# valette/FROG

Measured on AMD Instinct MI355X. Metric: registration iterations/sec (linear+deformable), higher is better.
Workload: dtype f32

## Files before the change

### frog_amd/csrc/device/ctx.h

```cpp
#pragma once

#include <hip/hip_runtime.h>

#include <cstdint>
#include <cstdio>
#include <cstring>
#include <string>
#include <memory>
#include <vector>

#include "../../../include/frog_hip.h"
#include "dev_buf.h"

namespace frog {

extern thread_local std::string g_last_error;

inline int fail(int code, const std::string &msg)
{
    g_last_error = msg;
    return code;
}

#define FROG_HIP_CHECK(expr)                                                            \
// ... 71 lines not shown
    std::shared_ptr<DevBuf<float4>> kept_u;
    std::shared_ptr<DevBuf<float4>> kept;
    bool retired = false;
};

}

struct frog_ctx {
    int device = 0;
    hipStream_t stream = nullptr;
    bool own_stream = false;
    frog_options opt{};

    uint32_t nI = 0, ib = 0, ie = 0;
    uint64_t P = 0;
    uint32_t own_pt_begin = 0, own_pt_end = 0;
    uint64_t L_own = 0;
    uint64_t L_recs = 0;
    std::vector<uint32_t> poff;
    std::vector<uint64_t> img_link_begin;

    frog::DevBuf<float4> pos;
    frog::DevBuf<frog::P3> pos2;
    frog::DevBuf<frog::P3> pos2_spec;
    frog::DevBuf<uint32_t> d_poff;
    frog::DevBuf<uint64_t> ref_rowptr;
    frog::DevBuf<uint32_t> ref_link;
    std::vector<uint32_t> h_old_of_new, h_new_of_old;
    frog::DevBuf<uint32_t> new_of_old;
    frog::DevBuf<frog::Tile> tiles;
    frog::DevBuf<frog::LinkRec> recs;
    frog::DevBuf<uint32_t> recs32;
    frog::RecFormat rec_format{};
    uint32_t n_tiles = 0;
    frog::DevBuf<uint32_t> img_tile_ptr;
    std::vector<uint32_t> h_img_tile_ptr;
    uint32_t n_sub = 1, n_groups = frog::N_XCD;
    uint32_t group_begin[frog::MAX_GROUPS + 1] = {};
    frog::DevBuf<double> tile_partial;
    frog::DevBuf<long long> tile_counts;
    frog::DevBuf<float4> group_sums;
    frog::DevBuf<float4> point_sums;
    frog::DevBuf<uint32_t> tile_order;
    frog::DevBuf<frog::Tile> tiles_bo;
    uint32_t n_order_blocks = 0;
    bool fused_sweep = false;
    bool fused_forced = false;

    frog::DevBuf<float4> em;
    frog::DevBuf<frog::EmDerived> emd;
    frog::DevBuf<frog::EmFast> emf;
    frog::DevBuf<float> samples;
    frog::DevBuf<unsigned char> em_guess;
    static constexpr int SEL_RING_MAX = 96;
    static constexpr int SEL_LOW_WATER = 3;
    int sel_ring = 2;
    frog::DevBuf<uint32_t> sample_ord[SEL_RING_MAX];
    frog::DevBuf<uint32_t> sample_count[SEL_RING_MAX];
    frog::DevBuf<uint2> sample_ends[SEL_RING_MAX];
    uint64_t sel_consumed = 0;
    uint64_t sel_produced = 0;
    int sel_used = 0;
    hipStream_t side = nullptr;
    hipStream_t setup_stream = nullptr;
    hipEvent_t setup_fork = nullptr, setup_join = nullptr;
    bool setup_pending = false;
    bool setup_deferred = false;
    hipEvent_t energy_copied = nullptr;
    bool xyz2_exported = false;
    hipEvent_t sel_done[SEL_RING_MAX] = {};
    hipEvent_t ord_read[SEL_RING_MAX] = {};
    frog::DevBuf<uint32_t> mt_state;
    std::vector<uint32_t> h_virtual;
    frog::DevBuf<uint32_t> d_virtual;
    int sample_cap = 0;

    frog::DevBuf<double> mat;
    frog::DevBuf<double> energy;
    frog::DevBuf<double> energy_blocks;
    frog::DevBuf<double> img_energy;
    frog::DevBuf<unsigned int> energy_ticket;
    double *h_energy = nullptr;
    double *h_energy_dev = nullptr;
    uint64_t scalar_seq = 0;

    bool deformable = false;
    frog::GridGeom geom{};
    frog::DevBuf<float4> coeff;
    frog::DevBuf<float4> grad;
    frog::DevBuf<float4> gradf;
    frog::DevBuf<float4> grad_spare;
    frog::DevBuf<uint32_t> lat_mask;
    frog::DevBuf<uint32_t> lat_inactive;
    frog::DevBuf<float4> ucoeff, ugrad, ugrad_spare;
    frog::DevBuf<double> gridsum;
    frog::DevBuf<uint32_t> perm;
    frog::DevBuf<uint32_t> key_ptr;
    frog::DevBuf<uint32_t> key_cursor;
    frog::DevBuf<uint32_t> key_counts, brick_ptr_scratch, scan_sums;
    frog::DevBuf<unsigned char> scatter_blocks;
    frog::DevBuf<unsigned char> scatter_blocks_tmp;
    frog::DevBuf<uint32_t> len_hist;
    uint32_t n_scatter_blocks = 0;
    frog::DevBuf<float> bounds_scratch;
    frog::DevBuf<unsigned int> stray;
    uint32_t stray_parity = 0;
// ... 110 lines not shown
```

### frog_amd/csrc/device/frog_hip.hip

```cpp

#include "ctx.h"
#include <hip/hip_ext.h>
#include "prep.h"
#include "k_links.hip.h"
#include "k_stats.hip.h"
#include "k_grid.hip.h"
#include "k_cull.hip.h"
#include "k_ransac.hip.h"
#include "k_reforder.hip.h"
#include "k_refchain.hip.h"
#include "similarity.h"

#include <atomic>
#include <chrono>
#include <cmath>
#include <cstdlib>
#include <random>
#include <limits>
#include <new>

namespace frog {
thread_local std::string g_last_error;
constexpr int BOUNDS_BLOCKS = 256;
void set_last_error(const std::string &s) { g_last_error = s; }
// ... 828 lines not shown
        const int n_slices = [&] {
            const char *e = getenv("FROG_TILE_SLICES");
            const int v = e ? atoi(e) : (c->ie - c->ib >= 64u ? 2 : 8);
            return v < 1 ? 1 : v > 64 ? 64 : v;
        }();
        for (int sl = 0; sl < n_slices; sl++)
            for (uint32_t i = c->ib; i < c->ie; i++) {
                const uint32_t tb = lay.img_tile_ptr[i], nt = lay.img_tile_ptr[i + 1] - tb;
                for (uint32_t j = 0; j < nt; j++)
                    if ((int)(((size_t)j * N_XCD * n_slices / nt) % n_slices) == sl) lists[(size_t)j * N_XCD / nt].push_back(tb + j);
            }
        size_t rounds = 0;
        for (auto &l : lists) rounds = std::max(rounds, l.size());
        std::vector<uint32_t> order(std::max<size_t>(1, rounds * N_XCD), 0xFFFFFFFFu);
        for (int x = 0; x < N_XCD; x++)
            for (size_t r = 0; r < lists[x].size(); r++) order[r * N_XCD + x] = lists[x][r];
        c->n_order_blocks = (uint32_t)(rounds * N_XCD);
        CREATE_CHECK(c->tile_order.upload(order, s));
        {
            std::vector<Tile> bo(order.size(), Tile{});
            for (size_t b = 0; b < order.size(); b++) if (order[b] != 0xFFFFFFFFu) bo[b] = lay.tiles[order[b]];
            CREATE_CHECK(c->tiles_bo.upload(bo, s));
            CREATE_CHECK(hipStreamSynchronize(s));
        }
        CREATE_CHECK(hipStreamSynchronize(s));
        uint32_t widest = 0;
        for (uint32_t g = 0; g < c->n_groups; g++) widest = std::max(widest, c->group_begin[g + 1] - c->group_begin[g]);
        const char *fe = getenv("FROG_SWEEP_FUSED");
        c->fused_sweep = c->n_sub == 1 && c->n_tiles > 0 && widest <= (uint32_t)EMD_LDS_IMAGES && sweep_lds_images(c) <= 64u
                         && !(fe && fe[0] == '0');
        c->fused_forced = fe && fe[0] == '1';
    }
    CREATE_CHECK(c->tile_partial.alloc((size_t)std::max(1u, c->n_tiles) * c->n_groups * LINEAR_SUMS));
    CREATE_CHECK(c->tile_counts.alloc((size_t)std::max(1u, c->n_tiles) * c->n_groups * 2));
    CREATE_CHECK(c->group_sums.alloc((size_t)N_XCD * std::max(1u, c->own_pt_end - c->own_pt_begin)));
    CREATE_CHECK(c->img_counts.alloc((size_t)c->n_owned() * 2));

    std::vector<float4> hem(c->nI, make_float4(10.f, 300.f, 0.5f, 0.f));
    CREATE_CHECK(c->em.upload(hem, s));
    CREATE_CHECK(c->emd.alloc(c->nI));
    CREATE_CHECK(c->emf.alloc(c->nI));
    c->h_virtual.resize(c->n_owned());
    uint32_t cap = 1;
    for (uint32_t i = c->ib; i < c->ie; i++) {
        uint64_t v = lay.img_link_begin[i + 1] - lay.img_link_begin[i];
        c->h_virtual[i - c->ib] = (uint32_t)v;
        cap = std::max<uint32_t>(cap, (uint32_t)std::min<uint64_t>(v, (uint64_t)o->stats_max_size));
    }
    c->sample_cap = (int)cap;
    CREATE_CHECK(c->d_virtual.upload(c->h_virtual, s));
    CREATE_CHECK(c->samples.alloc((size_t)c->n_owned() * cap));
    CREATE_CHECK(c->em_guess.alloc((size_t)c->n_owned() * 4 * EM_GUESS_BATCHES));
    CREATE_CHECK(hipMemsetAsync(c->em_guess.p, 0, c->em_guess.bytes(), s));
    c->sel_ring = 80;
    static_assert(80 <= frog_ctx::SEL_RING_MAX, "the ring's buffers are fixed arrays of frog_ctx");
    while (c->sel_ring > 2 && (size_t)c->sel_ring * c->n_owned() * cap * 12 > ((size_t)1 << 30)) c->sel_ring--;
    for (int b = 0; b < c->sel_ring; b++) {
        CREATE_CHECK(c->sample_ord[b].alloc((size_t)c->n_owned() * cap));
        CREATE_CHECK(c->sample_ends[b].alloc((size_t)c->n_owned() * cap));
        CREATE_CHECK(c->sample_count[b].alloc(c->n_owned()));
        CREATE_CHECK(hipMemsetAsync(c->sample_count[b].p, 0, c->sample_count[b].bytes(), s));
        CREATE_CHECK(hipEventCreateWithFlags(&c->ord_read[b], hipEventDisableTiming));
        CREATE_CHECK(hipEventCreateWithFlags(&c->sel_done[b], hipEventDisableTiming));
    }
    {
        int lo = 0, hi = 0;
        CREATE_CHECK(hipDeviceGetStreamPriorityRange(&lo, &hi));
        const bool high = c->sel_ring < 3;
        CREATE_CHECK(hipStreamCreateWithPriority(&c->side, hipStreamNonBlocking, high ? hi : lo));
    }
    CREATE_CHECK(hipEventCreateWithFlags(&c->energy_copied, hipEventDisableTiming));
    CREATE_CHECK(hipStreamCreateWithFlags(&c->setup_stream, hipStreamNonBlocking));
    CREATE_CHECK(hipEventCreateWithFlags(&c->setup_fork, hipEventDisableTiming));
    CREATE_CHECK(hipEventCreateWithFlags(&c->setup_join, hipEventDisableTiming));
    {
        std::vector<uint32_t> st((size_t)c->n_owned() * MT_WORDS);
        uint32_t x[MT_WORDS];
        x[0] = 0u;
        for (int k = 1; k < MT_N; k++) x[k] = 1812433253u * (x[k - 1] ^ (x[k - 1] >> 30)) + (uint32_t)k;
        x[MT_N] = MT_N;
        for (uint32_t i = 0; i < c->n_owned(); i++) std::memcpy(&st[(size_t)i * MT_WORDS], x, sizeof x);
        CREATE_CHECK(c->mt_state.upload(st, s));
    }

    std::vector<double> hm((size_t)c->nI * 16, 0.0);
    for (uint32_t i = 0; i < c->nI; i++) for (int k = 0; k < 4; k++) hm[(size_t)i * 16 + 5 * k] = 1.0;
    CREATE_CHECK(c->mat.upload(hm, s));
    CREATE_CHECK(c->energy.alloc(4));
    CREATE_CHECK(c->energy_blocks.alloc(2 * ENERGY_BLOCKS));
    CREATE_CHECK(c->img_energy.alloc(2 * (size_t)std::max(1u, c->n_owned())));
    CREATE_CHECK(c->energy_ticket.alloc(2));
    CREATE_CHECK(hipMemsetAsync(c->energy_ticket.p, 0, 2 * sizeof(unsigned int), s));
    CREATE_CHECK(hipMemsetAsync(c->energy.p, 0, c->energy.bytes(), s));
    CREATE_CHECK(c->stray.alloc(3));
    CREATE_CHECK(hipMemsetAsync(c->stray.p, 0, 3 * sizeof(unsigned int), s));
    CREATE_CHECK(c->bounds_scratch.alloc((size_t)BOUNDS_BLOCKS * 6 + 6));
    em_derive_kernel<<<div_up(c->nI, 256), 256, 0, s>>>(c->em.p, c->emd.p, c->emf.p, c->nI, c->fast_theta());
    CREATE_CHECK(hipGetLastError());
    if (const char *e = getenv("FROG_CULL")) c->cull_enabled = atoi(e) != 0;
    if (!(c->cull_enabled && c->opt.inlier_threshold >= 1e-3f) && !c->fused_forced) c->fused_sweep = false;
    if (const char *e = getenv("FROG_WEIGHT_EXACT")) c->exact_weights = atoi(e) != 0;
    if (const char *e = getenv("FROG_WEIGHT_GENERAL")) c->general_weights = atoi(e) != 0;
    c->ref_order = o->reference_order != 0;
    if (const char *e = getenv("FROG_REFERENCE_ORDER")) c->ref_order = atoi(e) != 0;
    if (const char *e = getenv("FROG_K11_F64")) c->k11_f64 = atoi(e) != 0;
    if (c->ref_order) { c->cull_enabled = false; c->exact_weights = true; c->fused_sweep = false; }
// ... 263 lines not shown
                                                                             ctx->perm.p, n, ctx->ib, to_dev(ctx->geom), apply,
                                                                             with_disp ? ctx->pos2_snap.p : nullptr, ctx->disp_part.p,
                                                                             after_step ? ctx->grad.p : nullptr, ctx->energy.p,
                                                                             ctx->opt.guarantee_diffeomorphism,
                                                                             ctx->disp_allow.p, ctx->cull_state.p, host_scalars, scalar_seq, trailer,
                                                                             pt_xcd ? nb : 0u);
            if (with_disp) ctx->disp_n = ctx->disp_own_n = div_up(n, 256);
        }
        trailer = nullptr;
        ctx->disp_others = false;
        if (out == ctx->pos2.p) ctx->disp_current = with_disp;
        else { ctx->disp_spec = with_disp; ctx->disp_current = false; }
    }
    if (trailer) slab_trailer_kernel<<<1, 1, 0, ctx->stream>>>(ctx->energy.p, trailer);
    FROG_HIP_CHECK(hipGetLastError());
    if (apply) { ctx->pos_b_stale = true; ctx->rc_valid = false; }
    return FROG_OK;
}

int frog_transform_points_local(frog_ctx *ctx, int apply)
{
    CTX_GUARD(ctx);
    const uint32_t n = ctx->own_pt_end - ctx->own_pt_begin;
    if (!n) return FROG_OK;
    if (ctx->xyz2_fresh && !apply) {
        ctx->xyz2_fresh = false; ctx->res_valid = false;
        ctx->disp_current = ctx->disp_spec;
        if (ctx->n_owned() == ctx->nI && !ctx->xyz2_exported && ctx->pos2_spec.n == ctx->pos2.n) {
            std::swap(ctx->pos2.p, ctx->pos2_spec.p);
            std::swap(ctx->pos2.cap, ctx->pos2_spec.cap);
            return FROG_OK;
        }
        FROG_HIP_CHECK(hipMemcpyAsync(ctx->pos2.p + ctx->own_pt_begin, ctx->pos2_spec.p + ctx->own_pt_begin,
                                      (size_t)n * sizeof(P3), hipMemcpyDeviceToDevice, ctx->stream));
        return FROG_OK;
    }
    ctx->xyz2_fresh = false; ctx->res_valid = false;
    return launch_transform(ctx, ctx->pos2.p, apply);
}

int frog_transform_points(frog_ctx *ctx, int apply) { return frog_transform_points_local(ctx, apply); }

int frog_update_stats_local(frog_ctx *ctx)
{
    CTX_GUARD(ctx);
    const uint32_t nO = ctx->n_owned();
    const uint32_t cap = (uint32_t)ctx->sample_cap;
    hipStream_t s = ctx->stream;
    const int cur = (int)(ctx->sel_consumed % (uint64_t)ctx->sel_ring);
    FROG_HIP_CHECK(hipStreamWaitEvent(s, ctx->sel_done[cur], 0));
    {
        Span span(ctx, FROG_K_STATS);
        sample_distance_kernel<<<dim3(div_up(cap, 256), nO), 256, 0, s>>>(
            ctx->sample_ends[cur].p, ctx->sample_count[cur].p, cap, ctx->pos2.p, ctx->samples.p);
        FROG_HIP_CHECK(hipGetLastError());
        em_scan_kernel<<<nO, EM_THREADS, 0, s>>>(ctx->samples.p, ctx->sample_count[cur].p, cap, ctx->ib, ctx->em.p,
                                                 ctx->opt.stats_max_iterations, ctx->opt.stats_epsilon, ctx->em_guess.p);
        FROG_HIP_CHECK(hipGetLastError());
    }
    FROG_HIP_CHECK(hipEventRecord(ctx->ord_read[cur], s));
    ctx->sel_used = cur;
    ctx->sel_consumed++;
    if (ctx->sel_produced - ctx->sel_consumed < (uint64_t)std::min((int)frog_ctx::SEL_LOW_WATER, ctx->sel_ring - 1))
        while (ctx->sel_produced - ctx->sel_consumed < (uint64_t)(ctx->sel_ring - 1)) {
            const int rc = produce_selection(ctx);
            if (rc) return rc;
            if (ctx->sel_ring > 8) break;
        }
    if (ctx->ib > 0) FROG_HIP_CHECK(hipMemsetAsync(ctx->em.p, 0, (size_t)ctx->ib * sizeof(float4), s));
    if (ctx->ie < ctx->nI)
        FROG_HIP_CHECK(hipMemsetAsync(ctx->em.p + ctx->ie, 0, (size_t)(ctx->nI - ctx->ie) * sizeof(float4), s));
    return FROG_OK;
}

int frog_stats_publish(frog_ctx *ctx)
{
    CTX_GUARD(ctx);
    stats_publish_kernel<<<dim3(div_up(ctx->nI, 64), 2), 64, 0, ctx->stream>>>(ctx->em.p, ctx->emd.p, ctx->emf.p, ctx->nI, ctx->opt.inlier_threshold, ctx->fast_theta(), ctx->cut_now.p,
                                                                       ctx->deformable ? 0 : 1);
    if (!ctx->deformable) ctx->cull_need_build = true;
    ctx->cull_check_due = true;
    FROG_HIP_CHECK(hipGetLastError());
    return FROG_OK;
}

int frog_update_stats(frog_ctx *ctx)
{
    if (ctx && !ctx->whole_group())
        return fail(FROG_E_STATE, "context owns a sub-range of images: use frog_update_stats_local + all-reduce + frog_stats_publish");
    int rc = frog_update_stats_local(ctx);
    if (rc) return rc;
    if (ctx->helper) {
        frog_ctx *h = ctx->helper;
        const size_t n = ctx->own_pt_end - ctx->own_pt_begin;
        FROG_HIP_CHECK(hipMemcpyAsync(h->pos2.p + ctx->own_pt_begin, ctx->pos2.p + ctx->own_pt_begin, n * sizeof(P3),
                                      hipMemcpyDeviceToDevice, ctx->stream));
        rc = frog_update_stats_local(h);
        if (rc) return rc;
        FROG_HIP_CHECK(hipMemcpyAsync(ctx->em.p, h->em.p, (size_t)ctx->nf * sizeof(float4), hipMemcpyDeviceToDevice, ctx->stream));
    }
    return frog_stats_publish(ctx);
}

int frog_ransac(frog_ctx *ctx, const frog_model *m, uint32_t image, const frog_ransac_options *o, int64_t *n_inliers)
{
    CTX_GUARD(ctx);
    if (!m || !o) return fail(FROG_E_INVALID, "null argument");
    if (image < ctx->ib || image >= ctx->ie) return fail(FROG_E_INVALID, "image not owned by this context");
    if (m->n_images != ctx->nI || m->point_offset[ctx->nI] != ctx->P) return fail(FROG_E_INVALID, "model does not match the context");
    if (ctx->deformable) return fail(FROG_E_STATE, "RANSAC after deformable set-up");
// ... 1048 lines not shown
    if (hipGetDeviceCount(&ndev) != hipSuccess || ndev < 1) return fail(FROG_E_NODEVICE, "no HIP device");
    if (device < 0 || device >= ndev) return fail(FROG_E_INVALID, "device index out of range");
    FROG_HIP_CHECK(hipSetDevice(device));
    if (!n) return FROG_OK;
    DevBuf<double> df, dw;
    FROG_HIP_CHECK(df.alloc(n)); FROG_HIP_CHECK(dw.alloc(4 * n));
    FROG_HIP_CHECK(hipMemcpy(df.p, f, n * sizeof(double), hipMemcpyHostToDevice));
    test_weights_kernel<<<div_up(n, 256), 256>>>(df.p, n, dw.p);
    FROG_HIP_CHECK(hipGetLastError());
    FROG_HIP_CHECK(hipMemcpy(out4n, dw.p, 4 * n * sizeof(double), hipMemcpyDeviceToHost));
    return FROG_OK;
}

int frog_test_cull_ranges(frog_ctx *ctx, uint64_t *ranges, uint64_t *with_election)
{
    CTX_GUARD(ctx);
    if (!ranges || !with_election) return fail(FROG_E_INVALID, "null output");
    *ranges = 0; *with_election = 0;
    if (ctx->cull_builds && ctx->act_cnt.n) {
        std::vector<uint32_t> h(ctx->act_cnt.n);
        FROG_HIP_CHECK(hipMemcpyAsync(h.data(), ctx->act_cnt.p, ctx->act_cnt.bytes(), hipMemcpyDeviceToHost, ctx->stream));
        FROG_HIP_CHECK(hipStreamSynchronize(ctx->stream));
        for (uint32_t v : h) {
            if (v & ~CULL_DUP_BIT) (*ranges)++;
            if (v & CULL_DUP_BIT) (*with_election)++;
        }
    }
    return FROG_OK;
}

int frog_test_stray_points(frog_ctx *ctx, uint64_t *n)
{
    CTX_GUARD(ctx);
    { const int rc_ = join_setup(ctx); if (rc_) return rc_; }
    if (!n) return fail(FROG_E_INVALID, "null output");
    unsigned int v = 0;
    FROG_HIP_CHECK(hipMemcpyAsync(&v, ctx->stray.p + 2, sizeof v, hipMemcpyDeviceToHost, ctx->stream));
    FROG_HIP_CHECK(hipStreamSynchronize(ctx->stream));
    *n = v;
    return FROG_OK;
}

int frog_test_em_refit(frog_ctx *ctx, int term_by_term)
{
    CTX_GUARD(ctx);
    const uint32_t nO = ctx->n_owned(), cap = (uint32_t)ctx->sample_cap;
    const int cur = ctx->sel_used;
    hipStream_t s = ctx->stream;
    if (term_by_term)
        em_kernel<<<nO, 256, 0, s>>>(ctx->samples.p, ctx->sample_count[cur].p, cap, ctx->ib, ctx->em.p,
                                     ctx->opt.stats_max_iterations, ctx->opt.stats_epsilon);
    else
        em_scan_kernel<<<nO, EM_THREADS, 0, s>>>(ctx->samples.p, ctx->sample_count[cur].p, cap, ctx->ib, ctx->em.p,
                                                 ctx->opt.stats_max_iterations, ctx->opt.stats_epsilon, nullptr);
    FROG_HIP_CHECK(hipGetLastError());
    return frog_stats_publish(ctx);
}

int frog_profile_enable(frog_ctx *ctx, int on)
{
    CTX_GUARD(ctx);
    ctx->profiling = (on == 2 || on == 3) ? 2 : (on != 0);
    ctx->profile_stride = on == 3 ? 4 : 1;
    return FROG_OK;
}

int frog_profile_read(frog_ctx *ctx, frog_kernel_time *out, int reset)
{
    CTX_GUARD(ctx);
    FROG_HIP_CHECK(hipStreamSynchronize(ctx->stream));
    for (auto &sp : ctx->spans) {
        float ms = 0.f;
        if (hipEventElapsedTime(&ms, sp.a, sp.b) == hipSuccess) {
            ctx->timed_ms[sp.slot] += (double)ms;
            ctx->timed_n[sp.slot] += 1;
        }
        ctx->free_events.emplace_back(sp.a, sp.b);
    }
    ctx->spans.clear();
    for (int k = 0; k < FROG_K_COUNT_; k++) {
        const uint64_t launches = ctx->timed_n[k] ? std::max(ctx->span_seen[k], ctx->timed_n[k]) : 0;
        ctx->ktime[k].launches = launches;
        ctx->ktime[k].ms_total = ctx->timed_n[k] ? ctx->timed_ms[k] / (double)ctx->timed_n[k] * (double)launches : 0.0;
    }
    if (out) std::memcpy(out, ctx->ktime, sizeof ctx->ktime);
    if (reset) {
        std::memset(ctx->ktime, 0, sizeof ctx->ktime);
        std::memset(ctx->span_seen, 0, sizeof ctx->span_seen);
        std::memset(ctx->timed_ms, 0, sizeof ctx->timed_ms);
        std::memset(ctx->timed_n, 0, sizeof ctx->timed_n);
    }
    return FROG_OK;
}

constexpr int UNPACK_MAX_RANKS = 64;
struct UnpackArgs {
    uint64_t row_begin[UNPACK_MAX_RANKS + 1];
    uint64_t slot_bytes;
    uint32_t world, self;
    uint64_t trailer_off;
    uint32_t sum_mask;
    double *energy, *host_scalars;
    double seq;
};
__global__ __launch_bounds__(256) void unpack_slab_kernel(const P3 *slab, P3 *pos2, const UnpackArgs a, const P3 *snap, uint32_t *disp_part)
{
    __shared__ uint32_t sh[4];
// ... 217 lines not shown
```

### frog_amd/csrc/device/k_stats.hip.h

```cpp
#pragma once

#include "ctx.h"

namespace frog {

constexpr int MT_N = 624;
constexpr int MT_M = 397;
constexpr int MT_WORDS = MT_N + 1;

__device__ __forceinline__ uint32_t mt_twist(uint32_t cur, uint32_t nxt, uint32_t far)
{
    uint32_t y = (cur & 0x80000000u) | (nxt & 0x7fffffffu);
    return far ^ (y >> 1) ^ ((y & 1u) ? 0x9908b0dfu : 0u);
}

constexpr int SELECT_THREADS = 256;

__device__ __forceinline__ void mt_regenerate(uint32_t *x, int tid)
{
    constexpr int LAG = MT_N - MT_M;
    uint32_t a = 0, b = 0, c = 0;
    if (tid < LAG) {
        a = mt_twist(x[tid], x[tid + 1], x[tid + MT_M]);
        b = mt_twist(x[tid + LAG], x[tid + LAG + 1], a);
// ... 87 lines not shown
            uint32_t rank = before + ((below_pk >> (8 * r)) & 0xFFu);
            #pragma unroll
            for (int w = 0; w < SELECT_THREADS / 64; w++) {
                const uint32_t c = row_cnt[r][w];
                if (w < wave) rank += c;
                before += c;
            }
            const uint32_t q = (uint32_t)tid + (uint32_t)(SELECT_THREADS * r);
            if (((keep_bits >> r) & 1u) && rank < need) ord[count + rank] = ordinal + q;
            if (((keep_bits >> r) & 1u) && fills && rank == need - 1) jstar_s = (int)q;
        }
        const bool advance = !fills && idx + n == (uint32_t)MT_N && ordinal + n < vs;
        if (advance && tid < LAG) {
            x[tid] = na;
            x[tid + LAG] = nb;
            if (tid + 2 * LAG < MT_N) x[tid + 2 * LAG] = nc;
        }
        __syncthreads();
        if (fills) {
            const uint32_t jstar = (uint32_t)jstar_s;
            idx += jstar + 1;
            ordinal += jstar + 1;
            count = cap;
            done = true;
        } else {
            count += kept;
            ordinal += n;
            idx = advance ? 0u : idx + n;
        }
    }
    for (int k = tid; k < MT_N; k += SELECT_THREADS) st[k] = x[k];
    if (tid == 0) { st[MT_N] = idx; sample_count[img] = count; }
}

__global__ __launch_bounds__(256) void sample_resolve_kernel(
    const uint32_t *sample_ord, const uint32_t *sample_count, uint32_t cap,
    const uint32_t *poff, uint32_t image_begin, uint32_t own_pt_begin,
    const uint64_t *ref_rowptr, const uint32_t *ref_link, const uint32_t *new_of_old, uint2 *sample_ends)
{
    const uint32_t img = blockIdx.y;
    const uint32_t slot = blockIdx.x * blockDim.x + threadIdx.x;
    if (slot >= sample_count[img]) return;
    const uint32_t image = image_begin + img;
    const uint32_t pb = poff[image] - own_pt_begin, pe = poff[image + 1] - own_pt_begin;
    const uint64_t l = ref_rowptr[pb] + sample_ord[(size_t)img * cap + slot];
    uint32_t lo = pb, hi = pe;
    while (hi - lo > 1) {
        uint32_t mid = (lo + hi) >> 1;
        if (ref_rowptr[mid] <= l) lo = mid; else hi = mid;
    }
    sample_ends[(size_t)img * cap + slot] = make_uint2(new_of_old[lo], ref_link[l]);
}

__global__ __launch_bounds__(256) void sample_distance_kernel(const uint2 *sample_ends, const uint32_t *sample_count, uint32_t cap,
                                                              const P3 *pos2, float *samples)
{
    const uint32_t img = blockIdx.y;
    const uint32_t slot = blockIdx.x * blockDim.x + threadIdx.x;
    if (slot >= sample_count[img]) return;
    const uint2 ends = sample_ends[(size_t)img * cap + slot];
    const P3 a = pos2[ends.x];
    const P3 b = pos2[ends.y];
    const float dx = a.x - b.x, dy = a.y - b.y, dz = a.z - b.z;
    samples[(size_t)img * cap + slot] = sqrtf(dx * dx + dy * dy + dz * dz);
}

__device__ __forceinline__ float chi_pdf_ref(float x)
{
    const float c = 0.797884560802865f;
    const float x2 = x * x;
    const float cx2 = c * x2;
    return (float)((double)cx2 * exp(-0.5 * (double)x2));
}

__device__ __forceinline__ float lane_f32(float v, int k)
{
    return __int_as_float(__builtin_amdgcn_readlane(__float_as_int(v), k));
}
__device__ __forceinline__ double lane_f64(double v, int k)
{
    const long long bits = __double_as_longlong(v);
    const int lo = __builtin_amdgcn_readlane((int)(bits & 0xffffffffll), k);
    const int hi = __builtin_amdgcn_readlane((int)(bits >> 32), k);
    return __longlong_as_double(((long long)hi << 32) | (unsigned int)lo);
}

__global__ __launch_bounds__(256) void em_kernel(const float *samples, const uint32_t *sample_count, uint32_t cap,
                                                 uint32_t image_begin, float4 *em, int max_iterations, float epsilon)
{
    __shared__ float t_s[2][64];
    __shared__ float sums_s[4];
    const uint32_t img = blockIdx.x;
    const uint32_t n = sample_count[img];
    const float *smp = samples + (size_t)img * cap;
    const int lane = threadIdx.x & 63, wave = threadIdx.x >> 6;
    const float4 e0 = em[image_begin + img];
    float c1 = e0.x, c2 = e0.y, ratio = e0.z;
    const float esp = 1.59576912160573f;
    const uint32_t n_batches = (n + 63) / 64;
    int iteration = 0;
    while (iteration++ < max_iterations) {
        auto membership = [&](uint32_t i) {
            float t = 0.f;
            if (i < n) {
                const float x = smp[i];
                const float f1 = ratio * chi_pdf_ref(x / c1) / c1;
                const float f2 = (float)((1.0 - (double)ratio) * (double)chi_pdf_ref(x / c2) / (double)c2);
                t = (float)((double)f1 / ((double)(f1 + f2) + 1e-16));
            }
            return t;
        };
        float sum1 = 0, sum2 = 0, sum3 = 0, sum4 = 0;
        if (wave == 3 && n_batches) t_s[0][lane] = membership(lane);
        __syncthreads();
        for (uint32_t b = 0; b < n_batches; b++) {
            const uint32_t base = b * 64;
            if (wave == 3) {
                if (b + 1 < n_batches) t_s[(b + 1) & 1][lane] = membership(base + 64 + lane);
            } else {
                const uint32_t i = base + lane;
                const float t = t_s[b & 1][lane];
                const float p = (i < n ? smp[i] : 0.f) * 1.0f;
                const int cnt = (int)min(64u, n - base);
                if (wave == 0) {
                    const float a = t * p;
// ... 110 lines not shown
                s = __builtin_ldexpf((float)(S + Pp), e - 23);
            }
        }
        if (stop < cnt) {
            const long long bits = __double_as_longlong(v);
            const int lo = __builtin_amdgcn_readlane((int)(bits & 0xffffffffll), stop);
            const int hi = __builtin_amdgcn_readlane((int)(bits >> 32), stop);
            const double vs = __longlong_as_double(((long long)hi << 32) | (unsigned int)lo);
            s = (float)((double)s + vs);
        }
        j = stop + 1;
    }
    return s;
}

__device__ __forceinline__ float em_chain_f32(float s, const float v, const int cnt, const int lane)
{
    int j = 0;
    while (j < cnt) {
        const uint32_t sb = __float_as_uint(s);
        const uint32_t ex = sb >> 23;
        const bool active = lane >= j && lane < cnt;
        int stop;
        if (ex == 0u || ex >= 255u) {
            if (sb == 0u) {
                const unsigned long long nz = __ballot(active && v != 0.0f);
                stop = nz ? (int)__ffsll((long long)nz) - 1 : cnt;
            } else {
                stop = j;
            }
        } else {
            const int e = (int)ex - 127;
            uint32_t r = 0;
            bool odd = false;
            if (active) r = em_term_f32(v, e, odd);
            const uint32_t P = wave_inclusive_scan_u32(r, lane);
            const uint32_t S = (sb & 0x7FFFFFu) | 0x800000u;
            const unsigned long long halt = __ballot(active && (odd || S + P >= 0x1000000u));
            stop = halt ? (int)__ffsll((long long)halt) - 1 : cnt;
            if (stop > j) {
                const uint32_t Pp = (uint32_t)__builtin_amdgcn_readlane((int)P, stop - 1);
                s = __builtin_ldexpf((float)(S + Pp), e - 23);
            }
        }
        if (stop < cnt) s += lane_f32(v, stop);
        j = stop + 1;
    }
    return s;
}

constexpr int EM_BATCHES = EM_CHUNK / 64;
constexpr int EM_GUESS_BATCHES = 1024;

__global__ __launch_bounds__(EM_THREADS) void em_scan_kernel(const float *samples, const uint32_t *sample_count, uint32_t cap,
                                                             uint32_t image_begin, float4 *em, int max_iterations, float epsilon,
                                                             unsigned char *guess_g )
{
    __shared__ float t_s[EM_CHUNK];
    __shared__ float p_s[EM_CHUNK];
    __shared__ float sums_s[4];
    __shared__ uint32_t total_s[4][EM_BATCHES];
    __shared__ unsigned char exact_s[4][EM_BATCHES];
    __shared__ unsigned char guess_s[4][EM_GUESS_BATCHES];
    const uint32_t img = blockIdx.x;
    const uint32_t n = sample_count[img];
    const float *smp = samples + (size_t)img * cap;
    const int lane = threadIdx.x & 63, wave = threadIdx.x >> 6;
    const float4 e0 = em[image_begin + img];
    float c1 = e0.x, c2 = e0.y, ratio = e0.z;
    const float esp = 1.59576912160573f;
    unsigned char *guess_mine = guess_g ? guess_g + (size_t)img * 4 * EM_GUESS_BATCHES : nullptr;
    for (int k = threadIdx.x; k < 4 * EM_GUESS_BATCHES; k += EM_THREADS) (&guess_s[0][0])[k] = guess_mine ? guess_mine[k] : 0;
    __syncthreads();
    int iteration = 0;
    while (iteration++ < max_iterations) {
        float sum1 = 0, sum2 = 0, sum3 = 0, sum4 = 0;
        for (uint32_t c0 = 0; c0 < n; c0 += EM_CHUNK) {
            const uint32_t m = min((uint32_t)EM_CHUNK, n - c0);
            const uint32_t gb0 = c0 / 64u;
            float x_next = (wave * 64u + lane) < m ? smp[c0 + wave * 64u + lane] : 0.f;
            for (uint32_t i0 = wave * 64u; i0 < m; i0 += EM_THREADS) {
                const uint32_t i = i0 + lane;
                const bool in = i < m;
                const float x = x_next;
                x_next = (i + EM_THREADS) < m ? smp[c0 + i + EM_THREADS] : 0.f;
                float t = 0.f, p = 0.f;
                if (in) {
                    const float f1 = ratio * chi_pdf_ref(x / c1) / c1;
                    const float f2 = (float)((1.0 - (double)ratio) * (double)chi_pdf_ref(x / c2) / (double)c2);
                    t = (float)((double)f1 / ((double)(f1 + f2) + 1e-16));
                    t_s[i] = t;
                    p = x * 1.0f;
                    p_s[i] = p;
                }
                const uint32_t lb = i0 / 64u, gb = gb0 + lb;
                #pragma unroll
                for (int a = 0; a < 4; a++) {
                    const uint32_t g = gb < (uint32_t)EM_GUESS_BATCHES ? guess_s[a][gb] : 0u;
                    uint32_t r = 0;
                    bool odd = false;
                    if (g - 1u < 254u && in) {
                        const int e = (int)g - 127;
                        if (a == 0) r = em_term_f32(t * p, e, odd);
                        else if (a == 1) r = em_term_f32(t, e, odd);
                        else if (a == 2) r = em_term_f64((1.0 - (double)t) * (double)p, e, odd);
                        else r = em_term_f64((1.0 - (double)t) * 1.0, e, odd);
                    }
                    const bool any_odd = __ballot(odd) != 0ull;
                    #pragma unroll
                    for (int off = 32; off > 0; off >>= 1) r += (uint32_t)__shfl_down((int)r, off, 64);
                    if (lane == 0) {
                        total_s[a][lb] = r;
                        exact_s[a][lb] = (g - 1u < 254u && !any_odd) ? 0 : 1;
                    }
                }
            }
            __syncthreads();
            if (wave < 4) {
                float acc = wave == 0 ? sum1 : wave == 1 ? sum2 : wave == 2 ? sum3 : sum4;
                const uint32_t n_b = (m + 63u) / 64u;
                uint32_t meta[2], tot[2], seen[2];
                #pragma unroll
                for (int h = 0; h < 2; h++) {
                    const uint32_t lb = (uint32_t)lane + 64u * h, gb = gb0 + lb;
                    const bool have = lb < n_b;
                    const uint32_t g = (have && gb < (uint32_t)EM_GUESS_BATCHES) ? guess_s[wave][gb] : 0u;
                    meta[h] = g | ((have ? (uint32_t)exact_s[wave][lb] : 1u) << 8);
                    tot[h] = have ? total_s[wave][lb] : 0u;
                    seen[h] = g;
                }
                for (uint32_t b = 0; b < m; b += 64) {
                    const uint32_t lb = b / 64u;
                    const uint32_t mt = (uint32_t)__builtin_amdgcn_readlane((int)(lb < 64u ? meta[0] : meta[1]), (int)(lb & 63u));
                    const uint32_t T = (uint32_t)__builtin_amdgcn_readlane((int)(lb < 64u ? tot[0] : tot[1]), (int)(lb & 63u));
                    const uint32_t sb = (uint32_t)__builtin_amdgcn_readfirstlane((int)__float_as_uint(acc));
                    const uint32_t ex = sb >> 23;
                    {
                        const uint32_t keep = ex < 255u ? ex : 0u;
                        if ((uint32_t)lane == (lb & 63u)) { if (lb < 64u) seen[0] = keep; else seen[1] = keep; }
                    }
                    if (mt == ex && ex - 1u < 254u) {
                        const uint32_t S = (sb & 0x7FFFFFu) | 0x800000u;
                        if (S + T < 0x1000000u) {
                            acc = __uint_as_float((ex << 23) | ((S + T) & 0x7FFFFFu));
                            continue;
                        }
                    }
                    const uint32_t i = b + lane;
                    const int cnt = (int)min(64u, m - b);
                    const float t = i < m ? t_s[i] : 0.f;
                    const float p = i < m ? p_s[i] : 0.f;
                    if (wave == 0) acc = em_chain_f32(acc, t * p, cnt, lane);
                    else if (wave == 1) acc = em_chain_f32(acc, t, cnt, lane);
                    else if (wave == 2) acc = em_chain(acc, (1.0 - (double)t) * (double)p, cnt, lane);
                    else acc = em_chain(acc, (1.0 - (double)t) * 1.0, cnt, lane);
                }
                if (wave == 0) sum1 = acc; else if (wave == 1) sum2 = acc; else if (wave == 2) sum3 = acc; else sum4 = acc;
                #pragma unroll
                for (int h = 0; h < 2; h++) {
                    const uint32_t lb = (uint32_t)lane + 64u * h, gb = gb0 + lb;
                    if (lb < n_b && gb < (uint32_t)EM_GUESS_BATCHES) guess_s[wave][gb] = (unsigned char)seen[h];
                }
            }
            __syncthreads();
        }
        if (lane == 0) {
            if (wave == 0) sums_s[0] = sum1;
            if (wave == 1) sums_s[1] = sum2;
            if (wave == 2) sums_s[2] = sum3;
            if (wave == 3) sums_s[3] = sum4;
        }
        __syncthreads();
        sum1 = sums_s[0]; sum2 = sums_s[1]; sum3 = sums_s[2]; sum4 = sums_s[3];
        __syncthreads();
        float sum5 = (float)n;
        sum2 = fmaxf(sum2, epsilon);
        sum3 = fmaxf(sum3, epsilon);
        sum5 = fmaxf(sum5, epsilon);
        const float nc1 = fmaxf(epsilon, sum1 / sum2 / esp);
        const float nc2 = fmaxf(epsilon, sum3 / sum4 / esp);
        const float nr = fmaxf(epsilon, sum2 / sum5);
        const bool done = (double)fabsf((c1 - nc1) / nc1) < 0.001
                       && (double)fabsf((c2 - nc2) / nc2) < 0.001
                       && (double)fabsf((nr - ratio) / nr) < 0.001;
        c1 = nc1; c2 = nc2; ratio = nr;
        if (done) break;
    }
    if (threadIdx.x == 0) em[image_begin + img] = make_float4(c1, c2, ratio, 0.f);
    if (guess_mine) {
        __syncthreads();
        for (int k = threadIdx.x; k < 4 * EM_GUESS_BATCHES; k += EM_THREADS) guess_mine[k] = (&guess_s[0][0])[k];
    }
}

__device__ __forceinline__ EmDerived em_derived_of(const float4 e)
{
    const float eps = 1e-10f;
    const float c = 0.797884560802865f;
    const float K = -0.72134752044448170368f;
    EmDerived d;
    const float inv1 = 1.0f / (e.x + eps), inv2 = 1.0f / (e.y + eps);
    const float q1 = inv1 * inv1, q2 = inv2 * inv2;
    d.kq1 = e.z * c * inv1 * q1;
    d.kq2 = (1.0f - e.z) * c * inv2 * q2;
    d.s1 = q1 * K;
    d.s2 = q2 * K;
    return d;
}

constexpr double EM_FAST_EPS_DROP = 7e-6;
constexpr double EM_FAST_DENSITY = 1e-10 / EM_FAST_EPS_DROP;
constexpr float EM_FAST_D2_MIN = 0.0100001f;

__device__ inline bool em_density_range(double kq, double s, double T, float &lo_out, float &hi_out)
{
    if (!(kq > 0.0) || !(kq < 1e30) || !(s < 0.0) || !(s > -1e30)) return false;
    const float kqf = (float)kq, sf = (float)s, Tf = (float)T;
    const float peak = -1.0f / (sf * 0.69314718f);
    auto xf = [&](float d2) { return kqf * d2 * __builtin_amdgcn_exp2f(sf * d2); };
    if (!(peak > 0.0f) || !(peak < 1e30f) || !(xf(peak) >= Tf)) return false;
    float a = 0.0f, b = peak;
    for (int k = 0; k < 26; k++) { const float m = 0.5f * (a + b); if (xf(m) >= Tf) b = m; else a = m; }
    const float lo = b * 1.001f;
    a = peak; b = peak;
    for (int k = 0; k < 12 && xf(b) >= Tf; k++) { a = b; b *= 4.0f; }
    if (xf(b) >= Tf) return false;
// ... 53 lines not shown
```

Measured before the change: 2406.

## Overlap EM chunk fill with chain reduction and precompute first EM pass

The EM scan kernel now double-buffers its shared chunk buffers. Waves beyond the four chain waves fill the next chunk's memberships and batch totals while the chain waves reduce the current chunk. The first iteration's memberships and per-batch totals are computed in the sample distance kernel, which has many more blocks, and stored to new global buffers that the scan kernel loads instead of recomputing. This costs extra global memory traffic and shared memory, and it shrinks the set of waves doing the fill.

Result: no change. 2420 (median of 5 runs) (+0.6%).

```diff
diff --git a/frog_amd/csrc/device/ctx.h b/frog_amd/csrc/device/ctx.h
--- a/frog_amd/csrc/device/ctx.h
+++ b/frog_amd/csrc/device/ctx.h
@@ -147,6 +147,9 @@
     frog::DevBuf<frog::EmFast> emf;
     frog::DevBuf<float> samples;
     frog::DevBuf<unsigned char> em_guess;
+    frog::DevBuf<float> em_t;
+    frog::DevBuf<uint32_t> em_total;
+    frog::DevBuf<unsigned char> em_exact;
     static constexpr int SEL_RING_MAX = 96;
     static constexpr int SEL_LOW_WATER = 3;
     int sel_ring = 2;
diff --git a/frog_amd/csrc/device/frog_hip.hip b/frog_amd/csrc/device/frog_hip.hip
--- a/frog_amd/csrc/device/frog_hip.hip
+++ b/frog_amd/csrc/device/frog_hip.hip
@@ -904,6 +904,9 @@
     CREATE_CHECK(c->samples.alloc((size_t)c->n_owned() * cap));
     CREATE_CHECK(c->em_guess.alloc((size_t)c->n_owned() * 4 * EM_GUESS_BATCHES));
     CREATE_CHECK(hipMemsetAsync(c->em_guess.p, 0, c->em_guess.bytes(), s));
+    CREATE_CHECK(c->em_t.alloc((size_t)c->n_owned() * cap));
+    CREATE_CHECK(c->em_total.alloc((size_t)c->n_owned() * 4 * div_up(cap, 64)));
+    CREATE_CHECK(c->em_exact.alloc((size_t)c->n_owned() * 4 * div_up(cap, 64)));
     c->sel_ring = 80;
     static_assert(80 <= frog_ctx::SEL_RING_MAX, "the ring's buffers are fixed arrays of frog_ctx");
     while (c->sel_ring > 2 && (size_t)c->sel_ring * c->n_owned() * cap * 12 > ((size_t)1 << 30)) c->sel_ring--;
@@ -1273,10 +1276,12 @@
     {
         Span span(ctx, FROG_K_STATS);
         sample_distance_kernel<<<dim3(div_up(cap, 256), nO), 256, 0, s>>>(
-            ctx->sample_ends[cur].p, ctx->sample_count[cur].p, cap, ctx->pos2.p, ctx->samples.p);
+            ctx->sample_ends[cur].p, ctx->sample_count[cur].p, cap, ctx->pos2.p, ctx->samples.p,
+            ctx->ib, ctx->em.p, ctx->em_guess.p, ctx->em_t.p, ctx->em_total.p, ctx->em_exact.p);
         FROG_HIP_CHECK(hipGetLastError());
         em_scan_kernel<<<nO, EM_THREADS, 0, s>>>(ctx->samples.p, ctx->sample_count[cur].p, cap, ctx->ib, ctx->em.p,
-                                                 ctx->opt.stats_max_iterations, ctx->opt.stats_epsilon, ctx->em_guess.p);
+                                                 ctx->opt.stats_max_iterations, ctx->opt.stats_epsilon, ctx->em_guess.p,
+                                                 ctx->em_t.p, ctx->em_total.p, ctx->em_exact.p);
         FROG_HIP_CHECK(hipGetLastError());
     }
     FROG_HIP_CHECK(hipEventRecord(ctx->ord_read[cur], s));
@@ -2431,7 +2436,8 @@
                                      ctx->opt.stats_max_iterations, ctx->opt.stats_epsilon);
     else
         em_scan_kernel<<<nO, EM_THREADS, 0, s>>>(ctx->samples.p, ctx->sample_count[cur].p, cap, ctx->ib, ctx->em.p,
-                                                 ctx->opt.stats_max_iterations, ctx->opt.stats_epsilon, nullptr);
+                                                 ctx->opt.stats_max_iterations, ctx->opt.stats_epsilon, nullptr,
+                                                 nullptr, nullptr, nullptr);
     FROG_HIP_CHECK(hipGetLastError());
     return frog_stats_publish(ctx);
 }
diff --git a/frog_amd/csrc/device/k_stats.hip.h b/frog_amd/csrc/device/k_stats.hip.h
--- a/frog_amd/csrc/device/k_stats.hip.h
+++ b/frog_amd/csrc/device/k_stats.hip.h
@@ -163,17 +163,31 @@
     sample_ends[(size_t)img * cap + slot] = make_uint2(new_of_old[lo], ref_link[l]);
 }
 
+__device__ __forceinline__ void em_first_pass(bool in, float x, size_t at, uint32_t img, uint32_t slot, uint32_t cap,
+                                              float4 e, const unsigned char *guess_g, float *t_g, uint32_t *total_g,
+                                              unsigned char *exact_g);
+
 __global__ __launch_bounds__(256) void sample_distance_kernel(const uint2 *sample_ends, const uint32_t *sample_count, uint32_t cap,
-                                                              const P3 *pos2, float *samples)
+                                                              const P3 *pos2, float *samples,
+                                                              uint32_t image_begin, const float4 *em, const unsigned char *guess_g,
+                                                              float *t_g, uint32_t *total_g, unsigned char *exact_g)
 {
     const uint32_t img = blockIdx.y;
     const uint32_t slot = blockIdx.x * blockDim.x + threadIdx.x;
-    if (slot >= sample_count[img]) return;
-    const uint2 ends = sample_ends[(size_t)img * cap + slot];
-    const P3 a = pos2[ends.x];
-    const P3 b = pos2[ends.y];
-    const float dx = a.x - b.x, dy = a.y - b.y, dz = a.z - b.z;
-    samples[(size_t)img * cap + slot] = sqrtf(dx * dx + dy * dy + dz * dz);
+    const uint32_t n = sample_count[img];
+    if ((slot & ~63u) >= n) return;
+    const bool in = slot < n;
+    const size_t at = (size_t)img * cap + slot;
+    float x = 0.f;
+    if (in) {
+        const uint2 ends = sample_ends[at];
+        const P3 a = pos2[ends.x];
+        const P3 b = pos2[ends.y];
+        const float dx = a.x - b.x, dy = a.y - b.y, dz = a.z - b.z;
+        x = sqrtf(dx * dx + dy * dy + dz * dz);
+        samples[at] = x;
+    }
+    em_first_pass(in, x, at, img, slot, cap, em[image_begin + img], guess_g, t_g, total_g, exact_g);
 }
 
 __device__ __forceinline__ float chi_pdf_ref(float x)
@@ -182,6 +196,13 @@
     const float x2 = x * x;
     const float cx2 = c * x2;
     return (float)((double)cx2 * exp(-0.5 * (double)x2));
+}
+
+__device__ __forceinline__ float em_membership(float x, float c1, float c2, float ratio)
+{
+    const float f1 = ratio * chi_pdf_ref(x / c1) / c1;
+    const float f2 = (float)((1.0 - (double)ratio) * (double)chi_pdf_ref(x / c2) / (double)c2);
+    return (float)((double)f1 / ((double)(f1 + f2) + 1e-16));
 }
 
 __device__ __forceinline__ float lane_f32(float v, int k)
@@ -398,126 +419,211 @@
 constexpr int EM_BATCHES = EM_CHUNK / 64;
 constexpr int EM_GUESS_BATCHES = 1024;
 
+__device__ __forceinline__ void em_batch_total(const int a, const uint32_t g, const bool in, const float t, const float p,
+                                               uint32_t &total, unsigned char &exact)
+{
+    uint32_t r = 0;
+    bool odd = false;
+    if (g - 1u < 254u && in) {
+        const int e = (int)g - 127;
+        if (a == 0) r = em_term_f32(t * p, e, odd);
+        else if (a == 1) r = em_term_f32(t, e, odd);
+        else if (a == 2) r = em_term_f64((1.0 - (double)t) * (double)p, e, odd);
+        else r = em_term_f64((1.0 - (double)t) * 1.0, e, odd);
+    }
+    const bool any_odd = __ballot(odd) != 0ull;
+    #pragma unroll
+    for (int off = 32; off > 0; off >>= 1) r += (uint32_t)__shfl_down((int)r, off, 64);
+    total = r;
+    exact = (g - 1u < 254u && !any_odd) ? 0 : 1;
+}
+
+__device__ __forceinline__ void em_first_pass(bool in, float x, size_t at, uint32_t img, uint32_t slot, uint32_t cap,
+                                              float4 e, const unsigned char *guess_g, float *t_g, uint32_t *total_g,
+                                              unsigned char *exact_g)
+{
+    float t = 0.f, p = 0.f;
+    if (in) {
+        t = em_membership(x, e.x, e.y, e.z);
+        t_g[at] = t;
+        p = x * 1.0f;
+    }
+    const uint32_t gb = slot / 64u, nb_cap = (cap + 63u) / 64u;
+    #pragma unroll
+    for (int a = 0; a < 4; a++) {
+        const uint32_t g = (guess_g && gb < (uint32_t)EM_GUESS_BATCHES)
+                               ? guess_g[((size_t)img * 4 + a) * EM_GUESS_BATCHES + gb] : 0u;
+        uint32_t total;
+        unsigned char exact;
+        em_batch_total(a, g, in, t, p, total, exact);
+        if ((threadIdx.x & 63) == 0) {
+            total_g[((size_t)img * 4 + a) * nb_cap + gb] = total;
+            exact_g[((size_t)img * 4 + a) * nb_cap + gb] = exact;
+        }
+    }
+}
+
+struct EmChunkBuf {
+    float *t, *p;
+    uint32_t (*total)[EM_BATCHES];
+    unsigned char (*exact)[EM_BATCHES];
+};
+
+__device__ __forceinline__ void em_fill_chunk(const EmChunkBuf buf, const unsigned char (*guess_s)[EM_GUESS_BATCHES], const float *smp,
+                                              const uint32_t c0, const uint32_t m, const float c1, const float c2, const float ratio,
+                                              const uint32_t w, const uint32_t n_waves, const int lane)
+{
+    const uint32_t gb0 = c0 / 64u;
+    const uint32_t stride = n_waves * 64u;
+    float x_next = (w * 64u + lane) < m ? smp[c0 + w * 64u + lane] : 0.f;
+    for (uint32_t i0 = w * 64u; i0 < m; i0 += stride) {
+        const uint32_t i = i0 + lane;
+        const bool in = i < m;
+        const float x = x_next;
+        x_next = (i + stride) < m ? smp[c0 + i + stride] : 0.f;
+        float t = 0.f, p = 0.f;
+        if (in) {
+            t = em_membership(x, c1, c2, ratio);
+            buf.t[i] = t;
+            p = x * 1.0f;
+            buf.p[i] = p;
+        }
+        const uint32_t lb = i0 / 64u, gb = gb0 + lb;
+        #pragma unroll
+        for (int a = 0; a < 4; a++) {
+            const uint32_t g = gb < (uint32_t)EM_GUESS_BATCHES ? guess_s[a][gb] : 0u;
+            uint32_t total;
+            unsigned char exact;
+            em_batch_total(a, g, in, t, p, total, exact);
+            if (lane == 0) {
+                buf.total[a][lb] = total;
+                buf.exact[a][lb] = exact;
+            }
+        }
+    }
+}
+
+__device__ __forceinline__ void em_load_chunk(const EmChunkBuf buf, const float *smp, const float *t_g, const uint32_t *total_g,
+                                              const unsigned char *exact_g, const uint32_t nb_cap, const uint32_t c0, const uint32_t m,
+                                              const uint32_t k, const uint32_t n_threads)
+{
+    for (uint32_t i = k; i < m; i += n_threads) {
+        buf.t[i] = t_g[c0 + i];
+        buf.p[i] = smp[c0 + i] * 1.0f;
+    }
+    const uint32_t gb0 = c0 / 64u, n_b = (m + 63u) / 64u;
+    for (uint32_t q = k; q < 4u * n_b; q += n_threads) {
+        const uint32_t a = q / n_b, lb = q - a * n_b;
+        buf.total[a][lb] = total_g[(size_t)a * nb_cap + gb0 + lb];
+        buf.exact[a][lb] = exact_g[(size_t)a * nb_cap + gb0 + lb];
+    }
+}
+
+__device__ __forceinline__ float em_chain_chunk(float acc, const int a, const EmChunkBuf buf, unsigned char (*guess_s)[EM_GUESS_BATCHES],
+                                                const uint32_t c0, const uint32_t m, const int lane)
+{
+    const uint32_t gb0 = c0 / 64u;
+    const uint32_t n_b = (m + 63u) / 64u;
+    uint32_t meta[2], tot[2], seen[2];
+    #pragma unroll
+    for (int h = 0; h < 2; h++) {
+        const uint32_t lb = (uint32_t)lane + 64u * h, gb = gb0 + lb;
+        const bool have = lb < n_b;
+        const uint32_t g = (have && gb < (uint32_t)EM_GUESS_BATCHES) ? guess_s[a][gb] : 0u;
+        meta[h] = g | ((have ? (uint32_t)buf.exact[a][lb] : 1u) << 8);
+        tot[h] = have ? buf.total[a][lb] : 0u;
+        seen[h] = g;
+    }
+    for (uint32_t b = 0; b < m; b += 64) {
+        const uint32_t lb = b / 64u;
+        const uint32_t mt = (uint32_t)__builtin_amdgcn_readlane((int)(lb < 64u ? meta[0] : meta[1]), (int)(lb & 63u));
+        const uint32_t T = (uint32_t)__builtin_amdgcn_readlane((int)(lb < 64u ? tot[0] : tot[1]), (int)(lb & 63u));
+        const uint32_t sb = (uint32_t)__builtin_amdgcn_readfirstlane((int)__float_as_uint(acc));
+        const uint32_t ex = sb >> 23;
+        {
+            const uint32_t keep = ex < 255u ? ex : 0u;
+            if ((uint32_t)lane == (lb & 63u)) { if (lb < 64u) seen[0] = keep; else seen[1] = keep; }
+        }
+        if (mt == ex && ex - 1u < 254u) {
+            const uint32_t S = (sb & 0x7FFFFFu) | 0x800000u;
+            if (S + T < 0x1000000u) {
+                acc = __uint_as_float((ex << 23) | ((S + T) & 0x7FFFFFu));
+                continue;
+            }
+        }
+        const uint32_t i = b + lane;
+        const int cnt = (int)min(64u, m - b);
+        const float t = i < m ? buf.t[i] : 0.f;
+        const float p = i < m ? buf.p[i] : 0.f;
+        if (a == 0) acc = em_chain_f32(acc, t * p, cnt, lane);
+        else if (a == 1) acc = em_chain_f32(acc, t, cnt, lane);
+        else if (a == 2) acc = em_chain(acc, (1.0 - (double)t) * (double)p, cnt, lane);
+        else acc = em_chain(acc, (1.0 - (double)t) * 1.0, cnt, lane);
+    }
+    #pragma unroll
+    for (int h = 0; h < 2; h++) {
+        const uint32_t lb = (uint32_t)lane + 64u * h, gb = gb0 + lb;
+        if (lb < n_b && gb < (uint32_t)EM_GUESS_BATCHES) guess_s[a][gb] = (unsigned char)seen[h];
+    }
+    return acc;
+}
+
 __global__ __launch_bounds__(EM_THREADS) void em_scan_kernel(const float *samples, const uint32_t *sample_count, uint32_t cap,
                                                              uint32_t image_begin, float4 *em, int max_iterations, float epsilon,
-                                                             unsigned char *guess_g )
-{
-    __shared__ float t_s[EM_CHUNK];
-    __shared__ float p_s[EM_CHUNK];
+                                                             unsigned char *guess_g ,
+                                                             const float *first_t ,
+                                                             const uint32_t *first_total, const unsigned char *first_exact)
+{
+    __shared__ float t_s[2][EM_CHUNK];
+    __shared__ float p_s[2][EM_CHUNK];
     __shared__ float sums_s[4];
-    __shared__ uint32_t total_s[4][EM_BATCHES];
-    __shared__ unsigned char exact_s[4][EM_BATCHES];
+    __shared__ uint32_t total_s[2][4][EM_BATCHES];
+    __shared__ unsigned char exact_s[2][4][EM_BATCHES];
     __shared__ unsigned char guess_s[4][EM_GUESS_BATCHES];
+    constexpr uint32_t CHAIN_WAVES = 4, ALL_WAVES = EM_THREADS / 64;
     const uint32_t img = blockIdx.x;
     const uint32_t n = sample_count[img];
     const float *smp = samples + (size_t)img * cap;
-    const int lane = threadIdx.x & 63, wave = threadIdx.x >> 6;
+    const int lane = threadIdx.x & 63;
+    const uint32_t wave = threadIdx.x >> 6;
     const float4 e0 = em[image_begin + img];
     float c1 = e0.x, c2 = e0.y, ratio = e0.z;
     const float esp = 1.59576912160573f;
+    const uint32_t nb_cap = (cap + 63u) / 64u;
+    const float *t_mine = first_t ? first_t + (size_t)img * cap : nullptr;
+    const uint32_t *total_mine = first_t ? first_total + (size_t)img * 4 * nb_cap : nullptr;
+    const unsigned char *exact_mine = first_t ? first_exact + (size_t)img * 4 * nb_cap : nullptr;
+    auto half = [&](const uint32_t h) { return EmChunkBuf{ t_s[h], p_s[h], total_s[h], exact_s[h] }; };
     unsigned char *guess_mine = guess_g ? guess_g + (size_t)img * 4 * EM_GUESS_BATCHES : nullptr;
     for (int k = threadIdx.x; k < 4 * EM_GUESS_BATCHES; k += EM_THREADS) (&guess_s[0][0])[k] = guess_mine ? guess_mine[k] : 0;
     __syncthreads();
+    const uint32_t n_chunks = (n + (uint32_t)EM_CHUNK - 1u) / (uint32_t)EM_CHUNK;
     int iteration = 0;
     while (iteration++ < max_iterations) {
-        float sum1 = 0, sum2 = 0, sum3 = 0, sum4 = 0;
-        for (uint32_t c0 = 0; c0 < n; c0 += EM_CHUNK) {
-            const uint32_t m = min((uint32_t)EM_CHUNK, n - c0);
-            const uint32_t gb0 = c0 / 64u;
-            float x_next = (wave * 64u + lane) < m ? smp[c0 + wave * 64u + lane] : 0.f;
-            for (uint32_t i0 = wave * 64u; i0 < m; i0 += EM_THREADS) {
-                const uint32_t i = i0 + lane;
-                const bool in = i < m;
-                const float x = x_next;
-                x_next = (i + EM_THREADS) < m ? smp[c0 + i + EM_THREADS] : 0.f;
-                float t = 0.f, p = 0.f;
-                if (in) {
-                    const float f1 = ratio * chi_pdf_ref(x / c1) / c1;
-                    const float f2 = (float)((1.0 - (double)ratio) * (double)chi_pdf_ref(x / c2) / (double)c2);
-                    t = (float)((double)f1 / ((double)(f1 + f2) + 1e-16));
-                    t_s[i] = t;
-                    p = x * 1.0f;
-                    p_s[i] = p;
-                }
-                const uint32_t lb = i0 / 64u, gb = gb0 + lb;
-                #pragma unroll
-                for (int a = 0; a < 4; a++) {
-                    const uint32_t g = gb < (uint32_t)EM_GUESS_BATCHES ? guess_s[a][gb] : 0u;
-                    uint32_t r = 0;
-                    bool odd = false;
-                    if (g - 1u < 254u && in) {
-                        const int e = (int)g - 127;
-                        if (a == 0) r = em_term_f32(t * p, e, odd);
-                        else if (a == 1) r = em_term_f32(t, e, odd);
-                        else if (a == 2) r = em_term_f64((1.0 - (double)t) * (double)p, e, odd);
-                        else r = em_term_f64((1.0 - (double)t) * 1.0, e, odd);
-                    }
-                    const bool any_odd = __ballot(odd) != 0ull;
-                    #pragma unroll
-                    for (int off = 32; off > 0; off >>= 1) r += (uint32_t)__shfl_down((int)r, off, 64);
-                    if (lane == 0) {
-                        total_s[a][lb] = r;
-                        exact_s[a][lb] = (g - 1u < 254u && !any_odd) ? 0 : 1;
-                    }
-                }
+        const bool ready = t_mine && iteration == 1;
+        auto fill = [&](const uint32_t c, const uint32_t w0) {
+            const uint32_t c0 = c * (uint32_t)EM_CHUNK, m = min((uint32_t)EM_CHUNK, n - c0);
+            if (ready) em_load_chunk(half(c & 1u), smp, t_mine, total_mine, exact_mine, nb_cap, c0, m, threadIdx.x - w0 * 64u, (ALL_WAVES - w0) * 64u);
+            else em_fill_chunk(half(c & 1u), guess_s, smp, c0, m, c1, c2, ratio, wave - w0, ALL_WAVES - w0, lane);
+        };
+        float acc = 0.f;
+        if (n_chunks) fill(0u, 0u);
+        __syncthreads();
+        for (uint32_t c = 0; c < n_chunks; c++) {
+            if (wave < CHAIN_WAVES) {
+                const uint32_t c0 = c * (uint32_t)EM_CHUNK, m = min((uint32_t)EM_CHUNK, n - c0);
+                if (wave == 0) acc = em_chain_chunk(acc, 0, half(c & 1u), guess_s, c0, m, lane);
+                else if (wave == 1) acc = em_chain_chunk(acc, 1, half(c & 1u), guess_s, c0, m, lane);
+                else if (wave == 2) acc = em_chain_chunk(acc, 2, half(c & 1u), guess_s, c0, m, lane);
+                else acc = em_chain_chunk(acc, 3, half(c & 1u), guess_s, c0, m, lane);
+            } else if (c + 1u < n_chunks) {
+                fill(c + 1u, CHAIN_WAVES);
             }
             __syncthreads();
-            if (wave < 4) {
-                float acc = wave == 0 ? sum1 : wave == 1 ? sum2 : wave == 2 ? sum3 : sum4;
-                const uint32_t n_b = (m + 63u) / 64u;
-                uint32_t meta[2], tot[2], seen[2];
-                #pragma unroll
-                for (int h = 0; h < 2; h++) {
-                    const uint32_t lb = (uint32_t)lane + 64u * h, gb = gb0 + lb;
-                    const bool have = lb < n_b;
-                    const uint32_t g = (have && gb < (uint32_t)EM_GUESS_BATCHES) ? guess_s[wave][gb] : 0u;
-                    meta[h] = g | ((have ? (uint32_t)exact_s[wave][lb] : 1u) << 8);
-                    tot[h] = have ? total_s[wave][lb] : 0u;
-                    seen[h] = g;
-                }
-                for (uint32_t b = 0; b < m; b += 64) {
-                    const uint32_t lb = b / 64u;
-                    const uint32_t mt = (uint32_t)__builtin_amdgcn_readlane((int)(lb < 64u ? meta[0] : meta[1]), (int)(lb & 63u));
-                    const uint32_t T = (uint32_t)__builtin_amdgcn_readlane((int)(lb < 64u ? tot[0] : tot[1]), (int)(lb & 63u));
-                    const uint32_t sb = (uint32_t)__builtin_amdgcn_readfirstlane((int)__float_as_uint(acc));
-                    const uint32_t ex = sb >> 23;
-                    {
-                        const uint32_t keep = ex < 255u ? ex : 0u;
-                        if ((uint32_t)lane == (lb & 63u)) { if (lb < 64u) seen[0] = keep; else seen[1] = keep; }
-                    }
-                    if (mt == ex && ex - 1u < 254u) {
-                        const uint32_t S = (sb & 0x7FFFFFu) | 0x800000u;
-                        if (S + T < 0x1000000u) {
-                            acc = __uint_as_float((ex << 23) | ((S + T) & 0x7FFFFFu));
-                            continue;
-                        }
-                    }
-                    const uint32_t i = b + lane;
-                    const int cnt = (int)min(64u, m - b);
-                    const float t = i < m ? t_s[i] : 0.f;
-                    const float p = i < m ? p_s[i] : 0.f;
-                    if (wave == 0) acc = em_chain_f32(acc, t * p, cnt, lane);
-                    else if (wave == 1) acc = em_chain_f32(acc, t, cnt, lane);
-                    else if (wave == 2) acc = em_chain(acc, (1.0 - (double)t) * (double)p, cnt, lane);
-                    else acc = em_chain(acc, (1.0 - (double)t) * 1.0, cnt, lane);
-                }
-                if (wave == 0) sum1 = acc; else if (wave == 1) sum2 = acc; else if (wave == 2) sum3 = acc; else sum4 = acc;
-                #pragma unroll
-                for (int h = 0; h < 2; h++) {
-                    const uint32_t lb = (uint32_t)lane + 64u * h, gb = gb0 + lb;
-                    if (lb < n_b && gb < (uint32_t)EM_GUESS_BATCHES) guess_s[wave][gb] = (unsigned char)seen[h];
-                }
-            }
-            __syncthreads();
-        }
-        if (lane == 0) {
-            if (wave == 0) sums_s[0] = sum1;
-            if (wave == 1) sums_s[1] = sum2;
-            if (wave == 2) sums_s[2] = sum3;
-            if (wave == 3) sums_s[3] = sum4;
-        }
-        __syncthreads();
-        sum1 = sums_s[0]; sum2 = sums_s[1]; sum3 = sums_s[2]; sum4 = sums_s[3];
+        }
+        if (lane == 0 && wave < CHAIN_WAVES) sums_s[wave] = acc;
+        __syncthreads();
+        float sum1 = sums_s[0], sum2 = sums_s[1], sum3 = sums_s[2], sum4 = sums_s[3];
         __syncthreads();
         float sum5 = (float)n;
         sum2 = fmaxf(sum2, epsilon);
```
